# spectralDNS/mpiFFT4py

Hardware: AMD Instinct MI355X
Metric: 3D R2C+C2R pairs/sec, 1024^3 fp64 slab (higher is better)
Workload: dtype f64; 1 GPU; 1024^3 fp64 slab R2C forward+inverse, device-resident, 1 rank(s); gpus_visible=1

## Files before the change

mpifft4py_amd/csrc/core.hip:

```cpp
#include <algorithm>
#include <cstdarg>
#include <type_traits>
#include <cstdio>
#include <cstdlib>
#include <map>
#include <mutex>
#include <unordered_map>
#include <tuple>
#include "mfft_internal.h"
#include "fft_nlz.h"

namespace mfft {

static thread_local std::string g_err;

int set_error(int code, const char* fmt, ...) {
  char buf[1024];
  va_list ap;
  va_start(ap, fmt);
  vsnprintf(buf, sizeof buf, fmt, ap);
  va_end(ap);
  g_err = buf;
  return code;
}
// ... 334 lines not shown
    e = find_chirpz(FAM_ROWZ, a.n, a.prec, inv);
    if (!e && big_length_ok(a.n)) return big_row(a, s);
    if (!e) return set_error(MFFT_ERR_UNSUPPORTED, "no kernel for a complex transform of length %d", a.n);
    MFFT_TRY(prepare_kernel(e, &tw));
    MFFT_TRY(chirpz_tables(a.n, e->n, a.prec, &chirp, &bhat));
    return by_prec(a.prec, [&](auto t) { return launch_row_t<decltype(t), RowParamsZ<decltype(t)>>(e, a, tw, s, chirp, bhat); });
  }
  MFFT_TRY(prepare_kernel(e, &tw));
  return by_prec(a.prec, [&](auto t) { return launch_row_t<decltype(t)>(e, a, tw, s); });
}

template <typename T, class PT = RealParams<T>>
static int launch_real_t(const KernelEntry* e, const RealArgs& a, void* tw, void* rtw, hipStream_t s,
                         const void* chirp = nullptr, const void* bhat = nullptr) {
  PT P;
  if constexpr (!std::is_same<PT, RealParams<T>>::value) {
    P.chirp = static_cast<const cx<T>*>(chirp);
    P.bhat = static_cast<const cx<T>*>(bhat);
    P.n = a.n;
  }
  P.in = a.in;
  P.out = a.out;
  P.tw = static_cast<const cx<T>*>(tw);
  P.rtw = static_cast<const cx<T>*>(rtw);
  P.in_stride = a.in_stride;
  P.out_stride = a.out_stride;
  P.nrows = a.nrows;
  P.valid = a.valid > 0 ? a.valid : a.n / 2 + 1;
  P.scale = (T)a.scale;
  if constexpr (std::is_same<PT, RealParams<T>>::value) set_zsplit(P, a.zs);
  return launch_rows(e, P, a.nrows, e->tile, s);
}
template <typename T>
static int launch_pair_t(const KernelEntry* e, const RealArgs& a, void* tw, void* rtw, hipStream_t s) {
  RealPairParams<T> P;
  P.in = a.in;
  P.out = a.out;
  P.tw = static_cast<const cx<T>*>(tw);
  P.rtw = static_cast<const cx<T>*>(rtw);
  P.in_stride = a.in_stride;
  P.out_stride = a.out_stride;
  P.nrows = (int64_t)(a.pair_n0 / 2 + 1) * a.pair_n1;
  P.valid = a.n / 2 + 1;
  P.scale = (T)a.scale;
  set_zsplit(P, a.zs);
  P.pn0 = a.pair_n0;
  P.pn1 = a.pair_n1;
  P.p_rplane = a.pair_rplane;
  P.p_cplane = a.pair_cplane;
  return launch_rows(e, P, P.nrows, e->tile / 2, s);
}

static int c2r_mlds_mode() {
  static const int m = getenv("MFFT_C2R_MLDS") ? atoi(getenv("MFFT_C2R_MLDS")) : 1;
  return m;
}
static bool c2r_mlds_take(int n, int prec, bool limited) {
  const int m = c2r_mlds_mode();
  if (m <= 0) return false;
  if (m == 2) return true;
  if (m == 3) return limited;
  const int c = n / 2;
  if (c == 1000 || c == 2000) return prec == MFFT_SINGLE;
  if (c == 1536) return limited && prec == MFFT_SINGLE;
  if (c == 2048) return !limited && prec == MFFT_DOUBLE;
  return true;
}
static int select_real(int fam, const RealArgs& a, const KernelEntry** out) {
  const bool limited = a.valid > 0 && a.valid < a.n / 2 + 1;
  const Op op = (limited ? Op::Limited : Op::Plain) | (a.zs.nchunk ? Op::ZChunk : Op::Plain);
  const KernelEntry* e = find_kernel(fam, a.n, a.prec, fam == FAM_C2R ? 1 : 0, op);
  if (fam == FAM_C2R && c2r_mlds_take(a.n, a.prec, limited))
    if (const KernelEntry* em = find_kernel(fam, a.n, a.prec, 1, op, Build::LdsMirrors)) e = em;
  const int64_t real_stride = fam == FAM_R2C ? a.in_stride : a.out_stride;
  if (a.zs.nchunk && (!e || real_stride % 2 != 0)) return set_error(MFFT_ERR_UNSUPPORTED, "no z-chunked real kernel of length %d", a.n);
  if (!e && limited) return set_error(MFFT_ERR_UNSUPPORTED, "no column-limited real kernel of length %d", a.n);
  if (!e || (real_stride % 2 != 0 && !limited)) {
    const bool r2c = fam == FAM_R2C;
    const bool half = a.n % 2 == 0 && a.n >= 4 && real_stride % 2 == 0;
    e = find_chirpz(half ? (r2c ? FAM_R2CZH : FAM_C2RZH) : (r2c ? FAM_R2CZ : FAM_C2RZ), half ? a.n / 2 : a.n, a.prec, r2c ? 0 : 1);
    if (!e && !big_length_ok(a.n)) return set_error(MFFT_ERR_UNSUPPORTED, "no kernel for a real transform of length %d", a.n);
  } else if (real_stride % 2 != 0) {
    return set_error(MFFT_ERR_UNSUPPORTED, "real row stride %lld must be even", (long long)real_stride);
  }
  *out = e;
  return 0;
}
bool pair_rows_supported(int64_t n, int prec) {
  return n >= 2 && n < 65536 && find_kernel(FAM_R2C, (int)n, prec, 0, Op::PairRows) && find_kernel(FAM_C2R, (int)n, prec, 1, Op::PairRows);
}
static int launch_real(int fam, const RealArgs& a, hipStream_t s) {
  const KernelEntry* e = nullptr;
  if (a.pair_n0 > 0) {
    e = find_kernel(fam, a.n, a.prec, fam == FAM_C2R ? 1 : 0, Op::PairRows);
    const int64_t real_stride = fam == FAM_R2C ? a.in_stride : a.out_stride;
    if (!e || a.zs.nchunk || a.valid > 0 || real_stride % 2 != 0 || a.pair_rplane % 2 != 0 ||
        a.nrows != (int64_t)a.pair_n0 * a.pair_n1 || a.nrows >= (int64_t)1 << 31)
      return set_error(MFFT_ERR_UNSUPPORTED, "no pair-row real kernel of length %d for this layout", a.n);
    void *tw = nullptr, *rtw = nullptr;
    MFFT_TRY(prepare_kernel(e, &tw));
    MFFT_TRY(real_twiddles(a.n, a.prec, &rtw));
    return by_prec(a.prec, [&](auto t) { return launch_pair_t<decltype(t)>(e, a, tw, rtw, s); });
  }
  MFFT_TRY(select_real(fam, a, &e));
  if (!e) return big_real(fam == FAM_C2R, a, s);
  void *tw = nullptr, *rtw = nullptr, *chirp = nullptr, *bhat = nullptr;
  MFFT_TRY(prepare_kernel(e, &tw));
  if (e->family != fam) {
    const bool half = e->family == FAM_R2CZH || e->family == FAM_C2RZH;
    MFFT_TRY(chirpz_tables(half ? a.n / 2 : a.n, e->n, a.prec, &chirp, &bhat));
    if (half) MFFT_TRY(real_twiddles(a.n, a.prec, &rtw));
    return by_prec(a.prec, [&](auto t) { return launch_real_t<decltype(t), RealParamsZ<decltype(t)>>(e, a, tw, rtw, s, chirp, bhat); });
  }
  MFFT_TRY(real_twiddles(a.n, a.prec, &rtw));
  return by_prec(a.prec, [&](auto t) { return launch_real_t<decltype(t)>(e, a, tw, rtw, s); });
}

int launch_r2c(const RealArgs& a, hipStream_t s) { return launch_real(FAM_R2C, a, s); }
int launch_c2r(const RealArgs& a, hipStream_t s) { return launch_real(FAM_C2R, a, s); }

static const KernelEntry* find_nlz(int64_t n, int prec, Op product, Build build = Build::Default) {
  const NlProduct& q = nl_product(product);
  if (n < 2 || n >= 65536 || (build == Build::AbsMax && !q.absmax) || (build == Build::Nlz3 && !q.nlz3)) return nullptr;
  return find_kernel(FAM_NLZ, (int)n, prec, 0, product, build);
}
bool nlz_supported(int64_t n, int prec, Op product, bool absmax) {
  if (absmax) return find_nlz(n, prec, product, Build::AbsMax) != nullptr;
  return find_nlz(n, prec, product) != nullptr || find_nlz(n, prec, product, Build::Nlz3) != nullptr;
}
int64_t nlz_absmax_waves(int64_t n, int prec, Op product, int64_t nrows) {
  const KernelEntry* e = find_nlz(n, prec, product, Build::AbsMax);
  if (!e || nrows < 1) return 0;
  return (nrows + 2 * e->tile - 1) / (2 * e->tile) * ((e->threads + 63) / 64);
}
template <typename T, class PT = NlzParams<T>>
// ... 284 lines not shown
```

mpifft4py_amd/csrc/fft_kernels.h:

```cpp
#pragma once
#include <type_traits>
#include "fft_core.h"

#if defined(__HIPCC__)
#define MFFT_D __device__ __forceinline__
#define MFFT_BARRIER() __syncthreads()
#if defined(__HIP_DEVICE_COMPILE__)
#define MFFT_OPAQUE(x) asm volatile("" : "+v"(x))
#else
#define MFFT_OPAQUE(x) ((void)0)
#endif
template <class S, bool ORIGIN = false> MFFT_D int row_thread_index(int tid) {
  int j = tid % S::TPT;
  if constexpr (::mfft::launder_plan<S>()) {
#if MFFT_LAUNDER_MODE == 1
    MFFT_OPAQUE(j);
#elif MFFT_LAUNDER_MODE == 4
    if constexpr (ORIGIN) MFFT_OPAQUE(j);
#endif
  }
  return j;
}
#else
#define MFFT_OPAQUE(x) ((void)0)
// ... 101 lines not shown
  int b_gzero;
  int in_wrap = 0, in_wrap_gap = 0;
};

template <typename T>
struct RowParams {
  const cx<T>* in;
  cx<T>* out;
  const cx<T>* tw;
  i64 in_stride, out_stride;
  i64 nrows;
  T scale;
  ZSplit zs;
  i64 row0;
};

template <typename T>
struct RealParams {
  const void* in;
  void* out;
  const cx<T>* tw;
  const cx<T>* rtw;
  i64 in_stride, out_stride;
  i64 nrows;
  int valid;
  T scale;
  ZSplit zs;
  i64 row0;
};
template <typename T>
struct RealPairParams : RealParams<T> {
  int pn0, pn1;
  i64 p_rplane, p_cplane;
};

struct PairRow {
  i64 real_off, cplx_off;
  bool live;
};
template <typename T>
MFFT_D PairRow pair_row(const RealPairParams<T>& P, i64 q, int side, i64 real_pitch, i64 cplx_pitch) {
  const bool inrange = q < P.nrows;
  if (!inrange) q = P.nrows - 1;
  const unsigned n0 = (unsigned)P.pn0, n1 = (unsigned)P.pn1;
  const unsigned kx = (unsigned)q / n1, ky = (unsigned)q - kx * n1;
  const unsigned px = kx ? n0 - kx : 0u, py = ky ? n1 - ky : 0u;
  bool live = inrange && !(px == kx && ky > py);
  if (side && px == kx && py == ky) live = false;
  const unsigned x = side ? px : kx, y = side ? py : ky;
  PairRow r;
  r.real_off = (i64)x * P.p_rplane + (i64)y * real_pitch;
  r.cplx_off = (i64)x * P.p_cplane + (i64)y * cplx_pitch;
  r.live = live;
  return r;
}

template <int PD> MFFT_HD int padpos(int pos) {
  if constexpr (PD > 0) return pos + pos / PD;
  else return pos;
}
template <int N, int PD> constexpr int padded_len() { return PD > 0 ? N + N / PD + 1 : N; }
template <int PD> struct PadSlot {
  MFFT_D int operator()(int pos) const { return padpos<PD>(pos); }
};

template <typename T, class Slot>
struct XchFull {
  cx<T>* buf;
  Slot slot;
  template <class S, int P>
  MFFT_D void exchange(cx<T> (&v)[S::E], int j, bool pre_barrier) {
    if (pre_barrier) MFFT_BARRIER();
    pass_scatter<S, P>(j, [&](int pos, int reg) { buf[slot(pos)] = v[reg]; });
    MFFT_BARRIER();
    pass_gather<S>(j, [&](int pos, int reg) { v[reg] = buf[slot(pos)]; });
  }
  MFFT_D void put(int pos, cx<T> val) { buf[slot(pos)] = val; }
  MFFT_D cx<T> get(int pos) { return buf[slot(pos)]; }
};

template <typename T, class Slot>
struct XchSplit {
  T* buf;
  Slot slot;
// ... 453 lines not shown
  typedef typename std::conditional<PAIR, RealPairParams<T>, RealParams<T>>::type Params;
  static constexpr int M = S::N;
  static constexpr int RPW = WP ? 64 / S::TPT : 1;
  static_assert(!WP || (S::TPT < 64 && 64 % S::TPT != 0 && ROWS % (64 / S::TPT) == 0), "wave-packed rows: whole waves of rows");
  static constexpr int THREADS = WP ? ROWS / RPW * 64 : S::TPT * ROWS;
  static constexpr int PD = S::R(0);
  static constexpr int PLEN = padded_len<M, PD>();
  static constexpr int TW_BYTES = TWLDS ? (int)(S::TW * sizeof(cx<T>)) : 0;
  static constexpr int XCH_BYTES = (int)(PLEN * ROWS * sizeof(XE));
  static constexpr int LDS_BYTES = TW_BYTES + XCH_BYTES;

  static MFFT_D void body(const Params& P, int bid, int tid, char* lds) {
    cx<T>* ltw = reinterpret_cast<cx<T>*>(lds);
    int rl, j, lane0 = 0;
    bool dup = false;
    if constexpr (WP) {
      const int lane = tid & 63;
      int lr = lane / S::TPT;
      dup = lr >= RPW;
      if (dup) lr = RPW - 1;
      lane0 = lr * S::TPT;
      j = dup ? lane - RPW * S::TPT : lane - lane0;
#if MFFT_LAUNDER_MODE == 1
      if constexpr (S::E % 15 == 0) MFFT_OPAQUE(j);
#endif
      rl = (tid >> 6) * RPW + lr;
    } else {
      rl = tid / S::TPT;
      j = row_thread_index<S>(tid);
    }
    XE* xch = reinterpret_cast<XE*>(lds + TW_BYTES) + rl * PLEN;
    const i64 row = (i64)bid * ROWS + rl;
    PairRow pr{};
    if constexpr (PAIR) pr = pair_row<T>(P, (i64)bid * (ROWS / 2) + (rl >> 1), rl & 1, P.in_stride, P.out_stride);
    const bool inrange = PAIR ? true : row < P.nrows;
    const bool active = PAIR ? pr.live : inrange && !dup;
    const cx<T>* ip =
        reinterpret_cast<const cx<T>*>(static_cast<const T*>(P.in) + (PAIR ? pr.real_off : (inrange ? row : P.nrows - 1) * P.in_stride));
    cx<T>* op = static_cast<cx<T>*>(P.out) + (PAIR ? pr.cplx_off : row * P.out_stride);

    cx<T> v[S::E];
#pragma unroll
    for (int k = 0; k < S::E; ++k) v[k] = ip[j + k * S::TPT];
    if constexpr (TWLDS && S::NP > 1) {
      stage_twiddles<S, T>(ltw, P.tw, tid, THREADS);
      MFFT_BARRIER();
    }
    typename RowXch<SPLIT, T, PadSlot<PD>>::type xc{xch, PadSlot<PD>{}};
    if constexpr (TWLDS) run_passes<S, 0, T>(v, j, (const cx<T>*)ltw, xc);
    else run_passes<S, 0, T>(v, j, P.tw, xc);

    const T half = (T)0.5;
    auto put = [&](int pos, cx<T> val) {
      if constexpr (CHUNK) {
        bool ok;
        const i64 o = zsplit_off(P.zs, P.row0 + row, pos, &ok);
        if (ok) static_cast<cx<T>*>(P.out)[o] = val;
      } else {
        op[pos] = val;
      }
    };
    auto emit_w = [&](int pos, cx<T> zk, cx<T> zpartner, cx<T> w) {
      if (pos == 0) {
        put(0, mk<T>((zk.x + zk.y) * P.scale, (T)0));
        if (!LIMIT || M < P.valid) put(M, mk<T>((zk.x - zk.y) * P.scale, (T)0));
      } else if (!LIMIT || pos < P.valid) {
        const cx<T> zm = conj(zpartner);
// ... 102 lines not shown
  typedef typename RowXch<SPLIT, T, PadSlot<S::R(0)>>::elem XE;
  static_assert(!PAIR || (!LIMIT && !CHUNK && !SPLIT && !WP && !MLDS && ROWS % 2 == 0 && S::NP > 1), "pair rows: plain dense kernels, whole pairs");
  typedef typename std::conditional<PAIR, RealPairParams<T>, RealParams<T>>::type Params;
  static constexpr int M = S::N;
  static constexpr int RPW = WP ? 64 / S::TPT : 1;
  static_assert(!WP || (S::TPT < 64 && 64 % S::TPT != 0 && ROWS % (64 / S::TPT) == 0), "wave-packed rows: whole waves of rows");
  static constexpr int THREADS = WP ? ROWS / RPW * 64 : S::TPT * ROWS;
  static constexpr int PD = S::R(0);
  static constexpr int PLEN = padded_len<M, PD>();
  static constexpr int TW_BYTES = TWLDS ? (int)(S::TW * sizeof(cx<T>)) : 0;
  static constexpr int XCH_BYTES = S::NP > 1 ? (int)(PLEN * ROWS * sizeof(XE)) : 0;
  static constexpr int LDS_BYTES = TW_BYTES + XCH_BYTES;

  static MFFT_D void body(const Params& P, int bid, int tid, char* lds) {
    cx<T>* ltw = reinterpret_cast<cx<T>*>(lds);
    int rl, j, lane0 = 0;
    bool dup = false;
    if constexpr (WP) {
      const int lane = tid & 63;
      int lr = lane / S::TPT;
      dup = lr >= RPW;
      if (dup) lr = RPW - 1;
      lane0 = lr * S::TPT;
      j = dup ? lane - RPW * S::TPT : lane - lane0;
      if constexpr (S::E % 15 == 0) MFFT_OPAQUE(j);
      rl = (tid >> 6) * RPW + lr;
    } else {
      rl = tid / S::TPT;
      j = row_thread_index<S, true>(tid);
    }
    XE* xch = reinterpret_cast<XE*>(lds + TW_BYTES) + rl * PLEN;
    const i64 row = (i64)bid * ROWS + rl;
    PairRow pr{};
    if constexpr (PAIR) pr = pair_row<T>(P, (i64)bid * (ROWS / 2) + (rl >> 1), rl & 1, P.out_stride, P.in_stride);
    const bool inrange = PAIR ? true : row < P.nrows;
    const bool active = PAIR ? pr.live : inrange && !dup;
    const cx<T>* ip = static_cast<const cx<T>*>(P.in) + (PAIR ? pr.cplx_off : (inrange ? row : P.nrows - 1) * P.in_stride);
    cx<T>* op = reinterpret_cast<cx<T>*>(static_cast<T*>(P.out) + (PAIR ? pr.real_off : row * P.out_stride));

    const i64 crow = P.row0 + (inrange ? row : P.nrows - 1);
    auto bin = [&](int pos) -> cx<T> {
      if constexpr (CHUNK) {
        bool ok;
        const i64 o = zsplit_off(P.zs, crow, pos, &ok);
        const cx<T> x = static_cast<const cx<T>*>(P.in)[ok ? o : (i64)0];
        if constexpr (sizeof(T) == 4) return keep_bits(x, ok);
        else return ok ? x : mk<T>((T)0, (T)0);
      } else {
        return ip[pos];
      }
    };
    cx<T> v[S::E];
    constexpr bool SHFL = WP || (S::TPT <= 64 && (64 % S::TPT) == 0);
    if constexpr (PAIR) {
      static_assert(PD > 0, "slot padpos(M) exists only in padded rows: PLEN = M + M / PD + 1");
#pragma unroll
      for (int k = 0; k < S::E; ++k) v[k] = ip[j + k * S::TPT];
      cx<T> xM = mk<T>((T)0, (T)0);
      if (j == 0) xM = ip[M];
      const XE* pxch = reinterpret_cast<const XE*>(lds + TW_BYTES) + (rl ^ 1) * PLEN;
#pragma unroll
      for (int k = 0; k < S::E; ++k) xch[padpos<PD>(j + k * S::TPT)] = v[k];
      if (j == 0) xch[padpos<PD>(M)] = xM;
      MFFT_BARRIER();
      const T half = (T)0.5;
#pragma unroll
      for (int k = 0; k < S::E; ++k) {
// ... 164 lines not shown
```

mpifft4py_amd/csrc/mfft_internal.h:

```cpp
#pragma once
#include <hip/hip_runtime.h>
#include <stdint.h>
#include <string>
#include <vector>
#include "../../include/mpifft4py_amd.h"
#include "registry.h"

namespace mfft {

int set_error(int code, const char* fmt, ...) __attribute__((format(printf, 2, 3)));
const char* last_error();

#define MFFT_HIP(call)                                                                   \
  do {                                                                                   \
    hipError_t e_ = (call);                                                              \
    if (e_ != hipSuccess)                                                                \
      return ::mfft::set_error(MFFT_ERR_HIP, "%s failed: %s (%s:%d)", #call,             \
                               hipGetErrorString(e_), __FILE__, __LINE__);               \
  } while (0)

#define MFFT_TRY(call)                  \
  do {                                  \
    int rc_ = (call);                   \
    if (rc_ != 0) return rc_;           \
// ... 37 lines not shown
int launch_col(const ColArgs& a, hipStream_t s);
bool mask_fusable(int64_t n, int prec);

struct ZSplitArgs {
  int nchunk = 0;
  int64_t q = 0, last_len = 0;
  int64_t rows_total = 0, row0 = 0;
  int64_t pitch = 0, last_pitch = 0;
};

struct RowArgs {
  const void* in = nullptr;
  void* out = nullptr;
  int n = 0;
  int prec = MFFT_DOUBLE;
  bool inverse = false;
  int64_t in_stride = 0, out_stride = 0, nrows = 0;
  double scale = 1.0;
  ZSplitArgs zs;
};
int launch_row(const RowArgs& a, hipStream_t s);

struct RealArgs {
  const void* in = nullptr;
  void* out = nullptr;
  int n = 0;
  int prec = MFFT_DOUBLE;
  int64_t in_stride = 0, out_stride = 0, nrows = 0;
  double scale = 1.0;
  int valid = 0;
  ZSplitArgs zs;
  int pair_n0 = 0, pair_n1 = 0;
  int64_t pair_rplane = 0, pair_cplane = 0;
};
int launch_r2c(const RealArgs& a, hipStream_t s);
int launch_c2r(const RealArgs& a, hipStream_t s);
bool pair_rows_supported(int64_t n, int prec);

struct NlzArgs {
  const void* a[3] = {nullptr, nullptr, nullptr};
  const void* b[3] = {nullptr, nullptr, nullptr};
  const void* c[3] = {nullptr, nullptr, nullptr};
  void* out[4] = {nullptr, nullptr, nullptr, nullptr};
  int n = 0;
  int prec = MFFT_DOUBLE;
  int64_t in_stride = 0, out_stride = 0, nrows = 0;
  int valid = 0;
  int valid_in = 0;
  double scale = 1.0;
  Op product = Op::Plain;
  void* part = nullptr;
};
struct NlProduct {
  Op op;
  const char* name;
  int nin, nout;
  bool absmax;
  bool nlz3;
};
constexpr NlProduct NL_PRODUCTS[] = {
    {Op::Plain, "cross", 6, 3, true, true},
    {Op::Dot, "dot", 6, 1, true, false},
    {Op::CrossDot, "cross_dot", 9, 4, false, false},
    {Op::Moments, "moments", 6, 0, false, false},
};
inline const NlProduct& nl_product(Op op) {
// ... 60 lines not shown
```

mpifft4py_amd/csrc/plan_create.hip:

```cpp
#include "plan_impl.h"

using namespace mfft;

#ifndef MFFT_DEFAULT_COMM_CUS
#define MFFT_DEFAULT_COMM_CUS 0
#endif

mfft_plan_s::~mfft_plan_s() {
  for (Buf* b : {&work[0], &work[1], &work[2], &work3, &nlw[0], &nlw[1], &nlx, &nly, &nlr, &pcomp, &shl, &nlm, &nlmacc, &nlsacc})
    if (b->p) (void)(b->arena ? wfree(b->p) : dev_free(b->p));
  if (mask) (void)hipFree(mask);
  if (band_tiles) (void)hipFree(band_tiles);
  for (auto& t : timers) {
    for (auto& e : t.pending) { (void)hipEventDestroy(e.first); (void)hipEventDestroy(e.second); }
    for (auto& e : t.pool) { (void)hipEventDestroy(e.first); (void)hipEventDestroy(e.second); }
  }
  drop_graphs();
  for (hipEvent_t e : ev_compute) (void)hipEventDestroy(e);
  for (hipEvent_t e : ev_comm) (void)hipEventDestroy(e);
  for (hipEvent_t e : ev2_compute) (void)hipEventDestroy(e);
  for (hipEvent_t e : ev2_comm) (void)hipEventDestroy(e);
  if (cstream) { big_release_stream(cstream); (void)hipStreamDestroy(cstream); }
  if (stream) { big_release_stream(stream); (void)hipStreamDestroy(stream); }
}
// ... 319 lines not shown
  MFFT_HIP(hipStreamSynchronize(p->stream));
  return 0;
}

static bool nonlinear_fused_key(mfft_plan_t p, const std::string& k, int64_t* value) {
  static const struct { const char* name; int mode; } modes[] = {{"none", MFFT_DEALIAS_NONE}, {"2_3", MFFT_DEALIAS_2_3}, {"3_2", MFFT_DEALIAS_3_2}};
  for (const NlProduct& q : NL_PRODUCTS) {
    const std::string named = q.op == Op::Plain ? "nonlinear" : std::string("nonlinear_") + q.name;
    for (int stats = 0; stats <= (q.absmax ? 1 : 0); ++stats)
      for (const auto& m : modes)
        if (k == named + (stats ? "_absmax" : "") + "_fused_" + m.name) {
          *value = p->nonlinear_fusable(m.mode, q.op, stats != 0) ? 1 : 0;
          return true;
        }
  }
  return false;
}

int mfft_plan_get_info(mfft_plan_t p, const char* key, int64_t* value) {
  if (!p || !key || !value) return set_error(MFFT_ERR_INVALID, "null argument");
  const std::string k(key);
  if (k == "pruned_route") *value = p->band_ok ? (p->band_allzero ? 2 : 1) : 0;
  else if (k == "local_band") *value = p->lband_ok ? 1 : 0;
  else if (k == "comm_cus") *value = p->comm_cus;
  else if (k == "kz_slices") *value = p->nslice;
  else if (k == "row_batches") *value = p->nbatch;
  else if (k == "zfuse") *value = p->zfuse ? 1 : 0;
  else if (k == "ranks") *value = p->P;
  else if (k == "complex_pitch") *value = p->pitched() ? p->Zp : 0;
  else if (k == "complex_pitch_native") *value = p->nat_pitch() ? 1 : 0;
  else if (nonlinear_fused_key(p, k, value)) return 0;
  else if (k == "nonlinear_bytes") *value = (int64_t)(p->nlx.bytes + p->nly.bytes + p->nlr.bytes + p->nlw[0].bytes + p->nlw[1].bytes);
  else if (k == "split_last") *value = p->split_last_route() ? 1 : 0;
  else if (k == "plane_pad") *value = (p->P == 1 && p->d.decomp == MFFT_SLAB) ? p->p1_plane_pad() : 0;
  else return set_error(MFFT_ERR_INVALID, "mfft_plan_get_info: unknown key '%s'", key);
  return 0;
}

int mfft_plan_timing(mfft_plan_t p, int enable) {
  if (!p) return set_error(MFFT_ERR_INVALID, "null plan");
  p->timing = enable != 0;
  return 0;
}

int mfft_plan_timing_reset(mfft_plan_t p) {
  if (!p) return set_error(MFFT_ERR_INVALID, "null plan");
  MFFT_TRY(p->collect_timing());
  for (auto& t : p->timers) {
    t.total_ms = 0;
    t.calls = 0;
  }
  return 0;
}

int mfft_plan_timing_get(mfft_plan_t p, int max_stages, char names[][32], double* total_ms, int64_t* calls, double* alg_bytes) {
  if (!p) return set_error(MFFT_ERR_INVALID, "null plan");
  MFFT_TRY(p->collect_timing());
  const int n = (int)p->timers.size();
  for (int i = 0; i < n && i < max_stages; ++i) {
    if (names) {
      strncpy(names[i], p->timers[i].name.c_str(), 31);
      names[i][31] = 0;
    }
    if (total_ms) total_ms[i] = p->timers[i].total_ms;
    if (calls) calls[i] = p->timers[i].calls;
    if (alg_bytes) alg_bytes[i] = p->timers[i].alg_bytes;
// ... 6 lines not shown
```

mpifft4py_amd/csrc/plan_impl.h:

```cpp
#pragma once
#include <algorithm>
#include <cmath>
#include <cstdlib>
#include <cstring>
#include <memory>
#include <string>
#include "comm.h"
#include "mfft_internal.h"

#ifndef MFFT_P1_XPAD_DEFAULT
#define MFFT_P1_XPAD_DEFAULT 0
#endif

namespace mfft {

inline bool env_on(const char* name) {
  const char* e = getenv(name);
  return e && atoi(e) != 0;
}
inline long env_int(const char* name, long dflt) {
  const char* e = getenv(name);
  return e ? atol(e) : dflt;
}

// ... 273 lines not shown
                                sc.part.empty() ? nullptr : sc.part.data());
  }
  void fill_part(bool comm0, std::vector<int>* part) const {
    part->resize(P);
    for (int r = 0; r < P; ++r) (*part)[r] = comm0 ? r / P1 : r % P1;
  }
  int xchg(int which, bool forward, bool padded, const void* send, void* recv) {
    Sched sc;
    MFFT_TRY(sched(which, forward, padded, &sc));
    return run_sched(sc, send, recv);
  }
  int sched_rows(int which, bool forward, int64_t i0, int64_t mb, Sched* out) const;
  int comm_waits(hipEvent_t e) {
    MFFT_HIP(hipEventRecord(e, stream));
    MFFT_HIP(hipStreamWaitEvent(cstream, e, 0));
    return 0;
  }
  int exchange_piece(const char* name, int which, bool forward, int piece, const void* send, void* recv, hipEvent_t done) {
    MFFT_TRY(stage_on(cstream, name, 0, [&] {
      Sched sc;
      MFFT_TRY(piece_sched(which, forward, piece, &sc));
      return run_sched(sc, send, recv, cstream);
    }));
    MFFT_HIP(hipEventRecord(done, cstream));
    return 0;
  }
  int npieces() const { return nbatch > 1 ? nbatch : nslice > 1 ? nslice : 1; }
  int piece_sched(int which, bool forward, int piece, Sched* out) const;

  bool fwd_out_of_place(size_t cbytes);
  int split_last = -1;
  int split_last_fit = -1;
  int64_t split_last_pad() const { return plane_pad(N1 * (N2 / 2)); }
  bool split_last_eligible() const;
  bool split_last_route();
  int slab_forward_split_last(const void* u, void* fu);
  int slab_backward_split_last(const void* fu, void* u);
  int slab_forward(const void* u, void* fu);
  int slab_backward(const void* fu, void* u, bool masked);
  int slab_backward_pruned(const void* fu, void* u);
  int slab_forward_pipelined(const void* u, void* fu);
  int slab_backward_pipelined(const void* src, void* u, bool pruned = false);
  int slab_forward_rows(const void* u, void* fu);
  int slab_backward_rows(const void* src, void* u, bool pruned = false);

  int pack_z(const void* Z, void* S, int64_t rows, int64_t nf, bool unpack);
  int pencil_forward_pipelined_x(const void* u, void* fu);
  int pencil_backward_pipelined_x(const void* src, void* u);
  int pencil_forward_pipelined_y(const void* u, void* fu);
  int pencil_backward_pipelined_y(const void* src, void* u);
  int pencil_forward(const void* u, void* fu);
  int pencil_backward(const void* fu, void* u, bool masked);

  bool band_ok = false;
  bool band_allzero = false;
  int ba0 = 0, bb0 = 0, ba1 = 0, bb1 = 0, ba2 = 0;
  int* band_tiles = nullptr;
  int band_ntiles = 0;
  bool lband_ok = false;
  int lb_row_lo = 0, lb_row_hi = 0, lb_g_lo = 0, lb_g_hi = 0, lb_c_lim = 0;
  const void* mask_src = nullptr;
  bool lband_use = false;
  bool prune_enabled() const { return !mfft::env_on("MFFT_NO_PRUNE"); }
  bool mask_set() const { return mask && mask_count == (size_t)local_complex_count(); }
  int require_mask() const {
    if (mask_set()) return 0;
    return mfft::set_error(MFFT_ERR_INVALID, "2/3-rule requested but no dealias mask of %zu entries was set", (size_t)local_complex_count());
  }
// ... 88 lines not shown
```

mpifft4py_amd/csrc/plan_sched.hip:

```cpp
#include "plan_impl.h"
#include "relay_plan.h"

using namespace mfft;

namespace {

std::vector<Chunk> pencil_chunks(int64_t n, int size) {
  std::vector<Chunk> c(size);
  const int64_t q = n / size, r = n % size;
  for (int i = 0; i < size; ++i) c[i] = Chunk{q + ((r == 1 && i == size - 1) ? 1 : 0), q * i};
  return c;
}

void compute_dims(int n, int* p1, int* p2) {
  int best1 = n, best2 = 1;
  for (int a = 1; a * a <= n; ++a)
    if (n % a == 0) {
      best1 = n / a;
      best2 = a;
    }
  *p1 = best1;
  *p2 = best2;
}

// ... 171 lines not shown
    else         { o->sd[g] = row; o->rd[g] = blk; }
  }
  return 0;
}

int mfft::decomp_init(mfft_plan_s* p, const mfft_plan_desc* desc, int nranks, int rank) {
  p->d = *desc;
  p->P = nranks;
  p->rank = rank;
  p->prec = desc->precision;
  p->r2c = desc->kind == MFFT_R2C;
  p->N0 = desc->n[0];
  p->N1 = desc->n[1];
  p->N2 = desc->n[2];
  if (nranks < 1 || rank < 0 || rank >= nranks) return set_error(MFFT_ERR_INVALID, "bad rank %d of %d", rank, nranks);
  if (p->N0 < 1 || p->N1 < 1 || p->N2 < 1) return set_error(MFFT_ERR_INVALID, "bad mesh");
  if (desc->precision != MFFT_SINGLE && desc->precision != MFFT_DOUBLE) return set_error(MFFT_ERR_INVALID, "bad precision");
  p->Nf = p->r2c ? p->N2 / 2 + 1 : p->N2;
  p->es = elem_bytes(p->prec, true);
  p->rs = p->r2c ? elem_bytes(p->prec, false) : p->es;
  const double ps = desc->padsize > 0 ? desc->padsize : 1.5;
  p->d.padsize = ps;
  p->M0 = (int64_t)(ps * p->N0);
  p->M1 = (int64_t)(ps * p->N1);
  p->M2 = (int64_t)(ps * p->N2);
  p->Mf = p->r2c ? (int64_t)(ps * p->N2) / 2 + 1 : p->M2;
  p->world.resize(p->P);
  for (int i = 0; i < p->P; ++i) p->world[i] = i;
  p->xpad_on = !env_on("MFFT_NO_XPAD");
  p->xpass_inplace = env_on("MFFT_XPASS_INPLACE");
  p->p1_xpad_lines = (int)env_int("MFFT_P1_XPAD", p->p1_xpad_lines);
  p->zpitch_on = !env_on("MFFT_NO_ZPITCH");
  if (getenv("MFFT_SPLIT_LAST")) p->split_last = env_on("MFFT_SPLIT_LAST") ? 1 : 0;
  if (getenv("MFFT_PAD_ALIGN")) p->pad_align = env_on("MFFT_PAD_ALIGN") ? 1 : 0;
  p->pad_align_inv = (int)env_int("MFFT_PAD_ALIGN_INV", p->pad_align_inv);
  const int P = p->P;
  if (p->r2c && p->N2 % 2) return set_error(MFFT_ERR_UNSUPPORTED, "odd N[2]=%lld is not supported for R2C", (long long)p->N2);
  p->Zp = 0;
  if (desc->decomp == MFFT_SLAB) {
    if (p->N0 % P || p->N1 % P) return set_error(MFFT_ERR_INVALID, "N[0]=%lld and N[1]=%lld must be divisible by the number of ranks %d", (long long)p->N0, (long long)p->N1, P);
    p->Np0 = p->N0 / P;
    p->Np1 = p->N1 / P;
    if (P > 1 && desc->pipeline < 0) {
      p->nbatch = (int)std::min<int64_t>(-(int64_t)desc->pipeline, p->Np0);
    } else if (P > 1) {
      const int want = desc->pipeline > 0 ? desc->pipeline : 4;
      const int64_t unit = 16;
      const int64_t per = (p->Nf / want) / unit * unit;
      if (want > 1 && per >= unit) {
        for (int s = 0; s < want; ++s) {
          const int64_t st = per * s;
          p->kslice.push_back(Chunk{s == want - 1 ? p->Nf - st : per, st});
        }
        p->nslice = want;
      }
    }
  } else if (desc->decomp == MFFT_PENCIL_X || desc->decomp == MFFT_PENCIL_Y) {
    int P1 = desc->p1, P2;
    if (P1 <= 0) compute_dims(P, &P1, &P2);
    else {
      if (P % P1) return set_error(MFFT_ERR_INVALID, "P1=%d does not divide %d ranks", P1, P);
      P2 = P / P1;
    }
    p->P1 = P1;
    p->P2 = P2;
    p->c0 = p->rank % P1;
// ... 112 lines not shown
```

mpifft4py_amd/csrc/plan_slab.hip:

```cpp
#include "plan_impl.h"

using namespace mfft;

#ifndef MFFT_FWD_OOP_DEFAULT
#define MFFT_FWD_OOP_DEFAULT 0
#endif

bool mfft_plan_s::fwd_out_of_place(size_t cbytes) {
  static const int mode = (int)env_int("MFFT_FWD_OOP", MFFT_FWD_OOP_DEFAULT);
  if (mode <= 0) return false;
  if (work[0].bytes >= cbytes) return true;
  size_t fr = 0, tot = 0;
  if (hipMemGetInfo(&fr, &tot) != hipSuccess) { (void)hipGetLastError(); return false; }
  return cbytes <= fr / 4;
}

bool mfft_plan_s::split_last_eligible() const {
  if (d.decomp != MFFT_SLAB || P != 1 || !r2c || nat_pitch() || d.line2d || d.drop_nyquist || split_last == 0) return false;
  if (N0 < 2 || N1 < 2 || N2 % 2 || !pair_rows_supported(N2, prec)) return false;
  if (split_last > 0) return true;
  return prec == MFFT_DOUBLE && N0 == 1024 && N1 == 1024 && N2 == 1024;
}
bool mfft_plan_s::split_last_route() {
  if (!split_last_eligible()) return false;
  if (split_last_fit < 0) {
    const size_t need = (size_t)(N0 * (N1 * (N2 / 2) + split_last_pad())) * es;
    size_t fr = 0, tot = 0;
    if (work[0].bytes >= need) split_last_fit = 1;
    else if (hipMemGetInfo(&fr, &tot) != hipSuccess) { (void)hipGetLastError(); split_last_fit = 0; }
    else split_last_fit = need <= fr / 4 ? 1 : 0;
  }
  return split_last_fit == 1;
}
int mfft_plan_s::slab_forward_split_last(const void* u, void* fu) {
  const int64_t M = N2 / 2, pl = N1 * M + split_last_pad();
  const double Wb = (double)(N0 * N1 * M) * es;
  MFFT_TRY(ensure(work[0], (size_t)(N0 * pl) * es));
  void* W = work[0].p;
  MFFT_TRY(stage("fwd_x", 2 * Wb, [&] { return col(u, W, N0, false, 1, N1 * M, 0, plain(N1 * M), 0, plain(pl)); }));
  MFFT_TRY(stage("fwd_y", 2 * Wb, [&] { return col(W, W, N1, false, N0, M, pl, plain(M), pl, plain(M)); }));
  return stage("fwd_z", Wb + (double)(N0 * N1 * Nf) * es, [&] {
    RealArgs a = real_args(W, fu, N0 * N1, N2, N2, Nf, 1.0);
    a.pair_n0 = (int)N0; a.pair_n1 = (int)N1; a.pair_rplane = 2 * pl; a.pair_cplane = N1 * Nf;
    return mfft::launch_r2c(a, stream);
  });
}
int mfft_plan_s::slab_backward_split_last(const void* fu, void* u) {
  const int64_t M = N2 / 2, pl = N1 * M + split_last_pad();
  const double Wb = (double)(N0 * N1 * M) * es;
  MFFT_TRY(ensure(work[0], (size_t)(N0 * pl) * es));
  void* W = work[0].p;
  MFFT_TRY(stage("bwd_z", Wb + (double)(N0 * N1 * Nf) * es, [&] {
    RealArgs a = real_args(fu, W, N0 * N1, N2, Nf, N2, 1.0 / (double)N2);
    a.pair_n0 = (int)N0; a.pair_n1 = (int)N1; a.pair_rplane = 2 * pl; a.pair_cplane = N1 * Nf;
    return mfft::launch_c2r(a, stream);
  }));
  MFFT_TRY(stage("bwd_y", 2 * Wb, [&] { return col(W, W, N1, true, N0, M, pl, plain(M), pl, plain(M)); }));
  return stage("bwd_x", 2 * Wb, [&] { return col(W, u, N0, true, 1, N1 * M, 0, plain(pl), 0, plain(N1 * M)); });
}

int mfft_plan_s::slab_forward(const void* u, void* fu) {
  const double Cb = (double)(N0 * Np1 * Nf) * es;
  const double Rb = (double)(Np0 * N1 * N2) * rs;
  if (P == 1 && split_last_route()) return slab_forward_split_last(u, fu);
  if (P == 1) {
    const int64_t Z = Zc();
    if (const int64_t xpad = p1_plane_pad()) {
      MFFT_TRY(stage("fwd_z", Rb + Cb, [&] { return z_forward(u, fu, N0 * N1, N2, Z); }));
      const int64_t pl = N1 * Z + xpad;
      MFFT_TRY(ensure(work[0], (size_t)(N0 * pl) * es));
      void* A = work[0].p;
      MFFT_TRY(stage("fwd_y", 2 * Cb, [&] { return col(fu, A, N1, false, N0, Nf, N1 * Z, plain(Z), pl, plain(Z)); }));
      MFFT_TRY(stage("fwd_x", 2 * Cb, [&] { return col(A, fu, N0, false, 1, N1 * Z, 0, plain(pl), 0, plain(N1 * Z)); }));
      return 0;
    }
    MFFT_TRY(stage("fwd_z", Rb + Cb, [&] { return z_forward(u, fu, N0 * N1, N2, Z); }));
    if (fwd_out_of_place((size_t)Cb)) {
      MFFT_TRY(ensure(work[0], (size_t)(N0 * N1 * Z) * es));
      void* A = work[0].p;
      MFFT_TRY(stage("fwd_y", 2 * Cb, [&] { return col(fu, A, N1, false, N0, Nf, N1 * Z, plain(Z), N1 * Z, plain(Z)); }));
      MFFT_TRY(stage("fwd_x", 2 * Cb, [&] { return col(A, fu, N0, false, 1, N1 * Z, 0, plain(N1 * Z), 0, plain(N1 * Z)); }));
      return 0;
    }
    MFFT_TRY(stage("fwd_y", 2 * Cb, [&] { return col(fu, fu, N1, false, N0, Nf, N1 * Z, plain(Z), N1 * Z, plain(Z)); }));
    MFFT_TRY(stage("fwd_x", 2 * Cb, [&] { return col(fu, fu, N0, false, 1, N1 * Z, 0, plain(N1 * Z), 0, plain(N1 * Z)); }));
    return 0;
  }
  if (nbatch > 1) return slab_forward_rows(u, fu);
  if (nslice > 1) return slab_forward_pipelined(u, fu);
  const int64_t S = Np1 * Nf + xplane_pad(true);
  const size_t cb = (size_t)std::max(Np0 * N1 * Nf, N0 * S) * es;
// ... 272 lines not shown
```

Baseline: 52.44 pairs/s.

## Add y-blocked workspace layout and y-first stage order to split-last slab path

Generalizes the split-last slab route's workspace layout so y rows can be grouped into blocks with separate row and block pitches, mapped in the pair-row real kernel through a row map. By default, on the 1024^3 double mesh, the y transform now runs first on the forward pass (and last on the backward pass) and uses a 16 KiB plane pad instead of the generic pad. The reordering changes which column pass touches user memory and how the strided passes hit memory channels. It adds extra index arithmetic in the kernel's real-offset computation.

```diff
diff --git a/mpifft4py_amd/csrc/core.hip b/mpifft4py_amd/csrc/core.hip
--- a/mpifft4py_amd/csrc/core.hip
+++ b/mpifft4py_amd/csrc/core.hip
@@ -390,7 +390,7 @@
   return launch_rows(e, P, a.nrows, e->tile, s);
 }
 template <typename T>
-static int launch_pair_t(const KernelEntry* e, const RealArgs& a, void* tw, void* rtw, hipStream_t s) {
+static int launch_pair_t(const KernelEntry* e, const RealArgs& a, int64_t real_stride, void* tw, void* rtw, hipStream_t s) {
   RealPairParams<T> P;
   P.in = a.in;
   P.out = a.out;
@@ -406,6 +406,7 @@
   P.pn1 = a.pair_n1;
   P.p_rplane = a.pair_rplane;
   P.p_cplane = a.pair_cplane;
+  P.p_ymap = make_rowmap(a.pair_rblock, real_stride, a.pair_yblock, a.pair_n1);
   return launch_rows(e, P, P.nrows, e->tile / 2, s);
 }
 
@@ -452,13 +453,15 @@
   if (a.pair_n0 > 0) {
     e = find_kernel(fam, a.n, a.prec, fam == FAM_C2R ? 1 : 0, Op::PairRows);
     const int64_t real_stride = fam == FAM_R2C ? a.in_stride : a.out_stride;
+    const bool blocked = a.pair_yblock > 0 && a.pair_yblock < a.pair_n1;
     if (!e || a.zs.nchunk || a.valid > 0 || real_stride % 2 != 0 || a.pair_rplane % 2 != 0 ||
-        a.nrows != (int64_t)a.pair_n0 * a.pair_n1 || a.nrows >= (int64_t)1 << 31)
+        a.nrows != (int64_t)a.pair_n0 * a.pair_n1 || a.nrows >= (int64_t)1 << 31 ||
+        (blocked && (a.pair_n1 >= 65536 || a.pair_n1 % a.pair_yblock != 0 || a.pair_rblock % 2 != 0)))
       return set_error(MFFT_ERR_UNSUPPORTED, "no pair-row real kernel of length %d for this layout", a.n);
     void *tw = nullptr, *rtw = nullptr;
     MFFT_TRY(prepare_kernel(e, &tw));
     MFFT_TRY(real_twiddles(a.n, a.prec, &rtw));
-    return by_prec(a.prec, [&](auto t) { return launch_pair_t<decltype(t)>(e, a, tw, rtw, s); });
+    return by_prec(a.prec, [&](auto t) { return launch_pair_t<decltype(t)>(e, a, real_stride, tw, rtw, s); });
   }
   MFFT_TRY(select_real(fam, a, &e));
   if (!e) return big_real(fam == FAM_C2R, a, s);
diff --git a/mpifft4py_amd/csrc/fft_kernels.h b/mpifft4py_amd/csrc/fft_kernels.h
--- a/mpifft4py_amd/csrc/fft_kernels.h
+++ b/mpifft4py_amd/csrc/fft_kernels.h
@@ -157,6 +157,7 @@
 struct RealPairParams : RealParams<T> {
   int pn0, pn1;
   i64 p_rplane, p_cplane;
+  RowMap p_ymap;
 };
 
 struct PairRow {
@@ -164,7 +165,7 @@
   bool live;
 };
 template <typename T>
-MFFT_D PairRow pair_row(const RealPairParams<T>& P, i64 q, int side, i64 real_pitch, i64 cplx_pitch) {
+MFFT_D PairRow pair_row(const RealPairParams<T>& P, i64 q, int side, i64 cplx_pitch) {
   const bool inrange = q < P.nrows;
   if (!inrange) q = P.nrows - 1;
   const unsigned n0 = (unsigned)P.pn0, n1 = (unsigned)P.pn1;
@@ -174,7 +175,7 @@
   if (side && px == kx && py == ky) live = false;
   const unsigned x = side ? px : kx, y = side ? py : ky;
   PairRow r;
-  r.real_off = (i64)x * P.p_rplane + (i64)y * real_pitch;
+  r.real_off = (i64)x * P.p_rplane + row_off(P.p_ymap, y);
   r.cplx_off = (i64)x * P.p_cplane + (i64)y * cplx_pitch;
   r.live = live;
   return r;
@@ -694,7 +695,7 @@
     XE* xch = reinterpret_cast<XE*>(lds + TW_BYTES) + rl * PLEN;
     const i64 row = (i64)bid * ROWS + rl;
     PairRow pr{};
-    if constexpr (PAIR) pr = pair_row<T>(P, (i64)bid * (ROWS / 2) + (rl >> 1), rl & 1, P.in_stride, P.out_stride);
+    if constexpr (PAIR) pr = pair_row<T>(P, (i64)bid * (ROWS / 2) + (rl >> 1), rl & 1, P.out_stride);
     const bool inrange = PAIR ? true : row < P.nrows;
     const bool active = PAIR ? pr.live : inrange && !dup;
     const cx<T>* ip =
@@ -863,7 +864,7 @@
     XE* xch = reinterpret_cast<XE*>(lds + TW_BYTES) + rl * PLEN;
     const i64 row = (i64)bid * ROWS + rl;
     PairRow pr{};
-    if constexpr (PAIR) pr = pair_row<T>(P, (i64)bid * (ROWS / 2) + (rl >> 1), rl & 1, P.out_stride, P.in_stride);
+    if constexpr (PAIR) pr = pair_row<T>(P, (i64)bid * (ROWS / 2) + (rl >> 1), rl & 1, P.in_stride);
     const bool inrange = PAIR ? true : row < P.nrows;
     const bool active = PAIR ? pr.live : inrange && !dup;
     const cx<T>* ip = static_cast<const cx<T>*>(P.in) + (PAIR ? pr.cplx_off : (inrange ? row : P.nrows - 1) * P.in_stride);
diff --git a/mpifft4py_amd/csrc/mfft_internal.h b/mpifft4py_amd/csrc/mfft_internal.h
--- a/mpifft4py_amd/csrc/mfft_internal.h
+++ b/mpifft4py_amd/csrc/mfft_internal.h
@@ -93,6 +93,8 @@
   ZSplitArgs zs;
   int pair_n0 = 0, pair_n1 = 0;
   int64_t pair_rplane = 0, pair_cplane = 0;
+  int pair_yblock = 0;
+  int64_t pair_rblock = 0;
 };
 int launch_r2c(const RealArgs& a, hipStream_t s);
 int launch_c2r(const RealArgs& a, hipStream_t s);
diff --git a/mpifft4py_amd/csrc/plan_create.hip b/mpifft4py_amd/csrc/plan_create.hip
--- a/mpifft4py_amd/csrc/plan_create.hip
+++ b/mpifft4py_amd/csrc/plan_create.hip
@@ -375,6 +375,11 @@
   else if (nonlinear_fused_key(p, k, value)) return 0;
   else if (k == "nonlinear_bytes") *value = (int64_t)(p->nlx.bytes + p->nly.bytes + p->nlr.bytes + p->nlw[0].bytes + p->nlw[1].bytes);
   else if (k == "split_last") *value = p->split_last_route() ? 1 : 0;
+  else if (k == "split_last_yblock") *value = p->split_last_route() ? p->split_last_layout().B : 0;
+  else if (k == "split_last_row_pitch") *value = p->split_last_route() ? p->split_last_layout().SR : 0;
+  else if (k == "split_last_block_pitch") *value = p->split_last_route() ? p->split_last_layout().SB : 0;
+  else if (k == "split_last_yfirst") *value = p->split_last_route() ? p->split_last_layout().yfirst : 0;
+  else if (k == "work_bytes") *value = (int64_t)p->work[0].bytes;
   else if (k == "plane_pad") *value = (p->P == 1 && p->d.decomp == MFFT_SLAB) ? p->p1_plane_pad() : 0;
   else return set_error(MFFT_ERR_INVALID, "mfft_plan_get_info: unknown key '%s'", key);
   return 0;
diff --git a/mpifft4py_amd/csrc/plan_impl.h b/mpifft4py_amd/csrc/plan_impl.h
--- a/mpifft4py_amd/csrc/plan_impl.h
+++ b/mpifft4py_amd/csrc/plan_impl.h
@@ -329,8 +329,22 @@
   int split_last = -1;
   int split_last_fit = -1;
   int64_t split_last_pad() const { return plane_pad(N1 * (N2 / 2)); }
+  int split_last_yblock = -1;
+  int split_last_yfirst = -1;
+  int64_t split_last_pad_bytes = -1;
+  struct SplitLastLayout {
+    int64_t B, SR, SB, nblk;
+    int yfirst;
+    bool yfirst_fwd() const { return yfirst > 0; }
+    bool yfirst_bwd() const { return yfirst == 1; }
+    int64_t elems() const { return nblk * SB; }
+  };
+  SplitLastLayout split_last_layout() const;
   bool split_last_eligible() const;
   bool split_last_route();
+  int split_last_x(const SplitLastLayout& l, const void* user_in, void* user_out, void* W, bool inv);
+  int split_last_y(const SplitLastLayout& l, const void* user_in, void* user_out, void* W, bool inv);
+  int split_last_z(const SplitLastLayout& l, const void* in, void* out, bool inv);
   int slab_forward_split_last(const void* u, void* fu);
   int slab_backward_split_last(const void* fu, void* u);
   int slab_forward(const void* u, void* fu);
diff --git a/mpifft4py_amd/csrc/plan_sched.hip b/mpifft4py_amd/csrc/plan_sched.hip
--- a/mpifft4py_amd/csrc/plan_sched.hip
+++ b/mpifft4py_amd/csrc/plan_sched.hip
@@ -227,6 +227,9 @@
   p->p1_xpad_lines = (int)env_int("MFFT_P1_XPAD", p->p1_xpad_lines);
   p->zpitch_on = !env_on("MFFT_NO_ZPITCH");
   if (getenv("MFFT_SPLIT_LAST")) p->split_last = env_on("MFFT_SPLIT_LAST") ? 1 : 0;
+  p->split_last_yblock = (int)env_int("MFFT_SPLIT_LAST_YBLOCK", p->split_last_yblock);
+  p->split_last_yfirst = (int)env_int("MFFT_SPLIT_LAST_YFIRST", p->split_last_yfirst);
+  p->split_last_pad_bytes = env_int("MFFT_SPLIT_LAST_PAD", p->split_last_pad_bytes);
   if (getenv("MFFT_PAD_ALIGN")) p->pad_align = env_on("MFFT_PAD_ALIGN") ? 1 : 0;
   p->pad_align_inv = (int)env_int("MFFT_PAD_ALIGN_INV", p->pad_align_inv);
   const int P = p->P;
diff --git a/mpifft4py_amd/csrc/plan_slab.hip b/mpifft4py_amd/csrc/plan_slab.hip
--- a/mpifft4py_amd/csrc/plan_slab.hip
+++ b/mpifft4py_amd/csrc/plan_slab.hip
@@ -21,10 +21,24 @@
   if (split_last > 0) return true;
   return prec == MFFT_DOUBLE && N0 == 1024 && N1 == 1024 && N2 == 1024;
 }
+mfft_plan_s::SplitLastLayout mfft_plan_s::split_last_layout() const {
+  const int64_t M = N2 / 2;
+  SplitLastLayout l;
+  l.B = N1;
+  if (split_last_yblock > 0 && split_last_yblock < N1 && N1 % split_last_yblock == 0 && N1 < 65536) l.B = split_last_yblock;
+  l.nblk = N1 / l.B;
+  const bool rule_mesh = prec == MFFT_DOUBLE && N0 == 1024 && N1 == 1024 && N2 == 1024;
+  l.yfirst = split_last_yfirst >= 0 ? std::min(split_last_yfirst, 2) : rule_mesh ? 1 : 0;
+  int64_t pad_r = l.B == N1 ? (rule_mesh && l.yfirst > 0 ? (int64_t)(16384 / es) : split_last_pad()) : slow_pitch_pad(l.B * M);
+  if (split_last_pad_bytes >= 0 && split_last_pad_bytes % 128 == 0) pad_r = split_last_pad_bytes / (int64_t)es;
+  l.SR = l.B * M + pad_r;
+  l.SB = N0 * l.SR + (l.nblk > 1 ? slow_pitch_pad(N0 * l.SR) : 0);
+  return l;
+}
 bool mfft_plan_s::split_last_route() {
   if (!split_last_eligible()) return false;
   if (split_last_fit < 0) {
-    const size_t need = (size_t)(N0 * (N1 * (N2 / 2) + split_last_pad())) * es;
+    const size_t need = (size_t)split_last_layout().elems() * es;
     size_t fr = 0, tot = 0;
     if (work[0].bytes >= need) split_last_fit = 1;
     else if (hipMemGetInfo(&fr, &tot) != hipSuccess) { (void)hipGetLastError(); split_last_fit = 0; }
@@ -32,31 +46,53 @@
   }
   return split_last_fit == 1;
 }
+int mfft_plan_s::split_last_x(const SplitLastLayout& l, const void* user_in, void* user_out, void* W, bool inv) {
+  const int64_t M = N2 / 2;
+  const void* in = user_in ? user_in : W;
+  void* out = user_out ? user_out : W;
+  return col(in, out, N0, inv, l.nblk, l.B * M, user_in ? l.B * M : l.SB, plain(user_in ? N1 * M : l.SR),
+             user_out ? l.B * M : l.SB, plain(user_out ? N1 * M : l.SR));
+}
+int mfft_plan_s::split_last_y(const SplitLastLayout& l, const void* user_in, void* user_out, void* W, bool inv) {
+  const int64_t M = N2 / 2;
+  const void* in = user_in ? user_in : W;
+  void* out = user_out ? user_out : W;
+  const RowSpec wrows = two_level(l.B, l.SB, M);
+  return col(in, out, N1, inv, N0, M, user_in ? N1 * M : l.SR, user_in ? plain(M) : wrows, user_out ? N1 * M : l.SR,
+             user_out ? plain(M) : wrows);
+}
+int mfft_plan_s::split_last_z(const SplitLastLayout& l, const void* in, void* out, bool inv) {
+  RealArgs a = inv ? real_args(in, out, N0 * N1, N2, Nf, N2, 1.0 / (double)N2) : real_args(in, out, N0 * N1, N2, N2, Nf, 1.0);
+  a.pair_n0 = (int)N0; a.pair_n1 = (int)N1; a.pair_rplane = 2 * l.SR; a.pair_cplane = N1 * Nf;
+  a.pair_yblock = (int)l.B; a.pair_rblock = 2 * l.SB;
+  return inv ? mfft::launch_c2r(a, stream) : mfft::launch_r2c(a, stream);
+}
 int mfft_plan_s::slab_forward_split_last(const void* u, void* fu) {
-  const int64_t M = N2 / 2, pl = N1 * M + split_last_pad();
-  const double Wb = (double)(N0 * N1 * M) * es;
-  MFFT_TRY(ensure(work[0], (size_t)(N0 * pl) * es));
+  const SplitLastLayout l = split_last_layout();
+  const double Wb = (double)(N0 * N1 * (N2 / 2)) * es;
+  MFFT_TRY(ensure(work[0], (size_t)l.elems() * es));
   void* W = work[0].p;
-  MFFT_TRY(stage("fwd_x", 2 * Wb, [&] { return col(u, W, N0, false, 1, N1 * M, 0, plain(N1 * M), 0, plain(pl)); }));
-  MFFT_TRY(stage("fwd_y", 2 * Wb, [&] { return col(W, W, N1, false, N0, M, pl, plain(M), pl, plain(M)); }));
-  return stage("fwd_z", Wb + (double)(N0 * N1 * Nf) * es, [&] {
-    RealArgs a = real_args(W, fu, N0 * N1, N2, N2, Nf, 1.0);
-    a.pair_n0 = (int)N0; a.pair_n1 = (int)N1; a.pair_rplane = 2 * pl; a.pair_cplane = N1 * Nf;
-    return mfft::launch_r2c(a, stream);
-  });
+  if (l.yfirst_fwd()) {
+    MFFT_TRY(stage("fwd_y", 2 * Wb, [&] { return split_last_y(l, u, nullptr, W, false); }));
+    MFFT_TRY(stage("fwd_x", 2 * Wb, [&] { return split_last_x(l, nullptr, nullptr, W, false); }));
+  } else {
+    MFFT_TRY(stage("fwd_x", 2 * Wb, [&] { return split_last_x(l, u, nullptr, W, false); }));
+    MFFT_TRY(stage("fwd_y", 2 * Wb, [&] { return split_last_y(l, nullptr, nullptr, W, false); }));
+  }
+  return stage("fwd_z", Wb + (double)(N0 * N1 * Nf) * es, [&] { return split_last_z(l, W, fu, false); });
 }
 int mfft_plan_s::slab_backward_split_last(const void* fu, void* u) {
-  const int64_t M = N2 / 2, pl = N1 * M + split_last_pad();
-  const double Wb = (double)(N0 * N1 * M) * es;
-  MFFT_TRY(ensure(work[0], (size_t)(N0 * pl) * es));
+  const SplitLastLayout l = split_last_layout();
+  const double Wb = (double)(N0 * N1 * (N2 / 2)) * es;
+  MFFT_TRY(ensure(work[0], (size_t)l.elems() * es));
   void* W = work[0].p;
-  MFFT_TRY(stage("bwd_z", Wb + (double)(N0 * N1 * Nf) * es, [&] {
-    RealArgs a = real_args(fu, W, N0 * N1, N2, Nf, N2, 1.0 / (double)N2);
-    a.pair_n0 = (int)N0; a.pair_n1 = (int)N1; a.pair_rplane = 2 * pl; a.pair_cplane = N1 * Nf;
-    return mfft::launch_c2r(a, stream);
-  }));
-  MFFT_TRY(stage("bwd_y", 2 * Wb, [&] { return col(W, W, N1, true, N0, M, pl, plain(M), pl, plain(M)); }));
-  return stage("bwd_x", 2 * Wb, [&] { return col(W, u, N0, true, 1, N1 * M, 0, plain(pl), 0, plain(N1 * M)); });
+  MFFT_TRY(stage("bwd_z", Wb + (double)(N0 * N1 * Nf) * es, [&] { return split_last_z(l, fu, W, true); }));
+  if (l.yfirst_bwd()) {
+    MFFT_TRY(stage("bwd_x", 2 * Wb, [&] { return split_last_x(l, nullptr, nullptr, W, true); }));
+    return stage("bwd_y", 2 * Wb, [&] { return split_last_y(l, nullptr, u, W, true); });
+  }
+  MFFT_TRY(stage("bwd_y", 2 * Wb, [&] { return split_last_y(l, nullptr, nullptr, W, true); }));
+  return stage("bwd_x", 2 * Wb, [&] { return split_last_x(l, nullptr, u, W, true); });
 }
 
 int mfft_plan_s::slab_forward(const void* u, void* fu) {
```

Result: faster. 53.49 pairs/s (median of 6 runs) (+2.0%).
